# Meng-333/FastDiffSR

Measured on NVIDIA B200. Metric: sr_images_per_s_T20, higher is better.
Workload: dtype fp16

## Files before the change

fastdiffsr_b200/csrc/api.cu:

```cuda
#include <algorithm>
#include <cmath>
#include <cstdarg>
#include <cstdio>
#include <cstdlib>
#include <cstring>
#include <map>
#include <string>
#include <utility>
#include <vector>

#include <cuda_runtime.h>

#include "../../include/fdsr.h"
#include "aux_kernels.cuh"
#include "conv_kernel.cuh"
#include "conv_f32.cuh"
#include "attn_kernel.cuh"
#include "tile_kernels.cuh"

using namespace fdsr;

namespace {

thread_local std::string g_global_error;
// ... 88 lines not shown
  std::string err;
  std::vector<HTensor> tensors;
  std::vector<HConv> convs;
  std::vector<HAttn> attns;
  std::vector<HOp> ops;
  int t_xin = -1, t_last = -1;
  std::map<std::string, std::vector<float>> host_w;
  bool weights_loaded = false;
  DevBuf<uint8_t> d_weights;
  DevBuf<float> d_params;
  DevBuf<float> d_bias;
  int T = 0;
  std::map<std::string, std::vector<double>> tables;
  std::vector<PostCoef> post;
  int B = 0, H = 0, W = 0;
  DevBuf<uint8_t> d_ws;
  size_t ws_bytes = 0;
  size_t stats_off = 0, stats_bytes = 0;
  size_t off_cond = 0, off_x = 0, off_eps = 0, off_sr = 0, off_psum = 0, off_pmax = 0, off_gate = 0,
         off_sp = 0, off_seed = 0;
  std::vector<ConvLayer> h_layers;
  std::vector<F32Layer> f_layers;
  std::vector<F32GnArgs> f_gn;
  std::vector<AttnParams> a_params;
  bool pair = true;
  bool half_tiles = true;
  bool split_n = true;
  bool epi2 = true;
  bool tail_help = true;
  bool resid_mma = true;
  bool up_phases = true;
  bool fused_tail = true;
  bool attn_ref = false;
  DevBuf<float> d_weights32;
  std::vector<size_t> w32_off;
  size_t off_gntab = 0;
  int esize() const { return cfg.dtype == FDSR_DTYPE_FP32 ? 4 : 2; }
  int bands() const { return cfg.out_channel; }
  DevBuf<long long> d_prof;
  bool layers_dirty = true;
  struct BicTab {
    int in, out, ksize;
    DevBuf<int> d_min, d_cnt, d_taps;
  };
  std::vector<BicTab> bic;
  DevBuf<uint8_t> d_bic_tmp;
  DevBuf<unsigned long long> d_metric;
  struct HostSlot {
    uint8_t* h_pin = nullptr;
    size_t h_pin_bytes = 0;
    DevBuf<uint8_t> d_stage;
    size_t in_b = 0, out_b = 0;
    cudaEvent_t computed = nullptr, copied = nullptr;
    bool busy = false;
  };
  static constexpr int kHostSlots = 2;
  HostSlot slot[kHostSlots];
  cudaStream_t copy_stream = nullptr;
  bool use_graph = true;
  DevBuf<PostStep> d_post;
  ConvLayer final_fused{};
  struct GraphEntry {
    int B, H, W;
    bool noise, trace;
    cudaGraphExec_t exec;
    uint64_t used;
// ... 50 lines not shown
}

template <typename... P, typename... A>
int launch(fdsr_ctx* c, void (*kernel)(P...), dim3 grid, dim3 block, size_t smem, cudaStream_t st, A&&... args) {
  kernel<<<grid, block, smem, st>>>(std::forward<A>(args)...);
  return launched(c, cudaSuccess, reinterpret_cast<const void*>(kernel));
}

template <typename T, typename H>
int upload(fdsr_ctx* c, DevBuf<T>& b, const std::vector<H>& host, size_t pad = 0) {
  cudaFree(b.ptr);
  b.ptr = nullptr;
  b.cap = 0;
  CUDA_TRY(c, b.grow(host.size() * sizeof(H) + pad));
  CUDA_TRY(c, cudaMemcpy(b.ptr, host.data(), host.size() * sizeof(H), cudaMemcpyHostToDevice));
  return FDSR_OK;
}

template <typename T>
struct Elem {
  using type = T;
};
template <typename F>
auto with_dtype16(const fdsr_ctx* c, F&& f) {
  return c->cfg.dtype == FDSR_DTYPE_BF16 ? f(Elem<__nv_bfloat16>{}) : f(Elem<__half>{});
}
template <typename F>
auto with_dtype(const fdsr_ctx* c, F&& f) {
  return c->cfg.dtype == FDSR_DTYPE_FP32 ? f(Elem<float>{}) : with_dtype16(c, f);
}

int pad_n(int cout) { return cout <= 16 ? 16 : (cout <= 64 ? 64 : (cout <= 128 ? 128 : 256)); }

constexpr int kOpScheduleFields = 17;

void add_conv(fdsr_ctx* c, const HConv& k) {
  c->convs.push_back(k);
  c->ops.push_back({0, int(c->convs.size()) - 1});
}

int add_tensor(fdsr_ctx* c, const std::string& name, int C, int level, bool stats) {
  HTensor t;
  t.name = name;
  t.C = C;
  t.level = level;
  t.stats = stats;
  c->tensors.push_back(t);
  return int(c->tensors.size()) - 1;
}

std::vector<HTap> taps3x3() {
  std::vector<HTap> v;
  for (int ky = 0; ky < 3; ++ky)
    for (int kx = 0; kx < 3; ++kx) v.push_back({ky, kx, ky * kPatchW + kx});
  return v;
}

int add_res(fdsr_ctx* c, const std::string& name, const std::vector<int>& srcs, int cout, int level,
            const std::string& out_name) {
  const std::string p = "denoise_fn." + name + ".res_block";
  int cin = 0;
  for (int s : srcs) cin += c->tensors[s].C;
  const int th = add_tensor(c, name + ".h", cout, level, true);
  const int to = add_tensor(c, out_name, cout, level, true);
  {
    HConv k;
    k.name = name + ".block1";
// ... 713 lines not shown
        g.C[s2] = t.C;
      }
      if (k.gn_nsrc == 1) {
        g.stats[1] = g.stats[0];
        g.C[1] = 0;
      }
      const HTensor& t0 = c->tensors[k.src[0]];
      g.gn_C = k.gn_C;
      g.groups = c->cfg.norm_groups;
      g.HW = (H >> t0.level) * (W >> t0.level);
      g.sq_scale = stat_sq_scale((long long)g.HW);
      g.eps = 1e-5f;
      g.gamma = c->d_params + k.gamma_off;
      g.beta = c->d_params + k.gamma_off + k.gn_C;
      g.tab = reinterpret_cast<float2*>(c->d_ws + c->off_gntab);
    }
  }
  static_assert(sizeof(F32Layer) <= 4000, "F32Layer must fit the kernel parameter space");
  c->layers_dirty = false;
  return FDSR_OK;
}

int launch_conv_f32(fdsr_ctx* c, int li, int t, cudaStream_t st) {
  const HConv& k = c->convs[li];
  const F32Layer& l = c->f_layers[li];
  if (k.gn_C) {
    const int rc = launch(c, f32_gn_table_kernel, c->B, 256, 0, st, c->f_gn[li]);
    if (rc) return rc;
  }
  const int tiles = c->B * ((l.W + kF32Tile - 1) / kF32Tile) * ((l.H + kF32Tile - 1) / kF32Tile);
  return launch(c, conv_f32_kernel, dim3(tiles, (l.N + kF32NBlk - 1) / kF32NBlk), 256, 0, st, l, t);
}

int upload_layers(fdsr_ctx* c) {
  if (c->cfg.dtype == FDSR_DTYPE_FP32) return upload_layers_f32(c);
  const int B = c->B, H = c->H, W = c->W;
  const bool bf = c->cfg.dtype == FDSR_DTYPE_BF16;
  if (!c->d_prof) {
    CUDA_TRY(c, c->d_prof.grow(size_t(c->num_sms) * kProfRoles * 64));
    CUDA_TRY(c, cudaMemset(c->d_prof, 0, size_t(c->num_sms) * kProfRoles * 64));
  }
  std::vector<ConvLayer> L(c->convs.size());
  for (size_t i = 0; i < c->convs.size(); ++i) {
    const HConv& k = c->convs[i];
    ConvLayer& l = L[i];
    memset(&l, 0, sizeof l);
    const int lvl = k.out >= 0 ? c->tensors[k.out].level : 0;
    l.B = B;
    l.phases = k.phases;
    l.H = (H >> lvl) >> (k.phases == 4 ? 1 : 0);
    l.W = (W >> lvl) >> (k.phases == 4 ? 1 : 0);
    l.tiles_x = (l.W + kTileW - 1) / kTileW;
    const int full_tiles = B * l.tiles_x * ((l.H + kTileH - 1) / kTileH);
    const bool half = c->half_tiles && c->pair && k.mode == kModeNormal && k.ncg == 8 && k.phases == 1 &&
                      k.out_mode == kOutAct && k.N >= 128 && l.tiles_x % 2 == 0 && l.H % 16 == 0 && full_tiles <= c->num_sms;
    l.tile_h = half ? 16 : kTileH;
    l.tiles_y = (l.H + l.tile_h - 1) / l.tile_h;
    l.ntiles = B * k.phases * l.tiles_x * l.tiles_y;
    l.nsplit = (!half && c->split_n && k.out_mode == kOutAct && k.N == 256 && 2 * l.ntiles <= c->num_sms) ? 2 : 1;
    l.n_full = k.N;
    l.N = k.N / l.nsplit;
    l.ncg = k.ncg;
    l.mode = k.mode;
    for (int s = 0; s < k.nsrc; ++s) {
      const HTensor& t = c->tensors[k.src[s]];
      l.src[s].ptr = c->d_ws + t.off;
// ... 53 lines not shown
      bool ok = true;
      if (k.phases == 4)
        for (int ph = 0; ph < 4 && ok; ++ph)
          ok = make_out_map_phase(ph == 0 ? &l.out_map : &l.out_map_ph[ph - 1], l.out, B, l.H, l.W, k.N, ph, bf);
      else if (k.N >= 32)
        ok = make_out_map(&l.out_map, l.out, B, l.H, l.W, k.N, bf);
      if (!ok) return fail(c, FDSR_E_CUDA, "layer %s: tensor maps of the output failed", k.name.c_str());
      l.out_stats = t.stats ? reinterpret_cast<unsigned long long*>(c->d_ws + t.stats_off) : nullptr;
      l.out_sq_scale = float(stat_sq_scale((long long)(H >> t.level) * (W >> t.level)));
      int su = 1;
      while (su < 8 && t.unit % (4 * su) == 0) su *= 2;
      l.out_su = (l.N == 64) ? 1 : su;
    } else {
      l.out = c->d_ws + c->off_eps;
    }
    l.pair = (c->pair && k.pair_ok() && l.a_tma && l.nsplit == 1 && l.tiles_x % 2 == 0) ? 1 : 0;
    l.weights = c->d_weights + (l.pair ? k.w_off2 : k.w_off);
    l.w_half = int32_t(k.w_bytes / 2);
    {
      const int tpi = l.tiles_x * l.tiles_y;
      l.group = (l.N == 64 && tpi % (l.pair ? 4 : 2) == 0) ? 2 : 1;
    }
    {
      bool raw = k.mode == kModeNormal && k.out_mode == kOutAct && l.tile_h == kTileH && l.nsplit == 1 && k.resid < 0;
      for (const HChunk& ch : k.chunks) raw = raw && ch.gn == 0;
      l.epi2 = (c->epi2 && raw) ? 1 : 0;
      if (l.epi2 && l.N <= 128) {
        l.nG = 2;
        l.nR = 0;
        for (int j = 0; j < l.nchunks; ++j) l.chunk[j].ring = 0;
      }
    }
    l.tail2 = (c->tail_help && !l.epi2 && k.out_mode == kOutAct && l.N >= 64) ? 1 : 0;
    l.prof = c->d_prof;
    l.flags = reinterpret_cast<unsigned int*>(c->d_ws + kOffFlags);
  }
  static_assert(sizeof(ConvLayer) <= 4000, "ConvLayer must fit the kernel parameter space");
  c->final_fused = L.back();
  c->final_fused.out_mode = kOutPosterior;
  c->final_fused.post = c->d_post;
  c->final_fused.x_state = reinterpret_cast<float*>(c->d_ws + c->off_x);
  c->final_fused.xin = c->d_ws + c->tensors[c->t_xin].off;
  c->final_fused.args = reinterpret_cast<const SampleArgs*>(c->d_ws + c->off_seed);
  c->h_layers = L;
  const int rc = upload_attn(c);
  if (rc) return rc;
  c->layers_dirty = false;
  return FDSR_OK;
}

int ensure_layers(fdsr_ctx* c) { return c->layers_dirty ? upload_layers(c) : FDSR_OK; }

template <int N, typename T>
cudaError_t set_conv_attr() {
  cudaError_t e = cudaFuncSetAttribute(conv_gemm_kernel<N, T, false>, cudaFuncAttributeMaxDynamicSharedMemorySize,
                                       ConvCfg<N>::kSmemBytes);
  if constexpr (N >= 64) {
    if (e == cudaSuccess)
      e = cudaFuncSetAttribute(conv_gemm_kernel<N, T, true>, cudaFuncAttributeMaxDynamicSharedMemorySize,
                               ConvCfg<N>::kSmemBytes);
  }
  return e;
}
template <typename T>
cudaError_t set_conv_attrs() {
  cudaError_t e = set_conv_attr<16, T>();
// ... 418 lines not shown
  return launch(c, set_args_kernel, 1, 1, 0, st, reinterpret_cast<SampleArgs*>(c->d_tiled.ptr),
                SampleArgs{seed, c->image0, noise, trace});
}
}

extern "C" {

const char* fdsr_global_error(void) { return g_global_error.c_str(); }
const char* fdsr_last_error(const fdsr_ctx* ctx) { return ctx ? ctx->err.c_str() : g_global_error.c_str(); }

int fdsr_create(const fdsr_config* cfg, fdsr_ctx** out) {
  if (!cfg || !out) return fail(nullptr, FDSR_E_INVALID, "null argument");
  int ndev = 0;
  if (cudaGetDeviceCount(&ndev) != cudaSuccess || ndev == 0)
    return fail(nullptr, FDSR_E_CUDA, "no CUDA device: libfdsr has no CPU fallback");
  fdsr_ctx* c = new fdsr_ctx();
  c->cfg = *cfg;
  cudaGetDevice(&c->device);
  cudaDeviceProp prop;
  if (cudaGetDeviceProperties(&prop, c->device) != cudaSuccess || prop.major != 10) {
    delete c;
    return fail(nullptr, FDSR_E_CUDA, "libfdsr needs an sm_100 (B200) device");
  }
  c->num_sms = prop.multiProcessorCount;
  c->pair = env_hook("FDSR_PAIR", c->pair);
  c->half_tiles = env_hook("FDSR_HALF_TILES", c->half_tiles);
  c->split_n = env_hook("FDSR_SPLIT_N", c->split_n);
  c->epi2 = env_hook("FDSR_EPI2", c->epi2);
  c->tail_help = env_hook("FDSR_TAIL_HELP", c->tail_help);
  c->resid_mma = env_hook("FDSR_RESID_MMA", c->resid_mma);
  c->up_phases = env_hook("FDSR_UP_PHASES", c->up_phases);
  c->fused_tail = env_hook("FDSR_FUSED_TAIL", c->fused_tail);
  c->attn_ref = env_hook("FDSR_ATTN_REF", c->attn_ref);
  if (cfg->dtype < FDSR_DTYPE_FP16 || cfg->dtype > FDSR_DTYPE_FP32) {
    delete c;
    return fail(nullptr, FDSR_E_INVALID, "dtype must be FDSR_DTYPE_FP16, FDSR_DTYPE_BF16 or FDSR_DTYPE_FP32");
  }
  const int rc = build_plan(c);
  if (rc) {
    g_global_error = c->err;
    delete c;
    return rc;
  }
  const cudaError_t ae = cfg->dtype == FDSR_DTYPE_FP32 ? cudaSuccess : with_dtype16(c, [&](auto e) {
    using T = typename decltype(e)::type;
    cudaError_t r = set_conv_attrs<T>();
    for (const HAttn& a : c->attns)
      if (r == cudaSuccess && a.kind == 1)
        r = cudaFuncSetAttribute(attn_core<T>(a.C).first, cudaFuncAttributeMaxDynamicSharedMemorySize,
                                 attn_core<T>(a.C).second);
    return r;
  });
  if (ae != cudaSuccess) {
    delete c;
    return fail(nullptr, FDSR_E_CUDA, "cudaFuncSetAttribute(max dynamic smem) failed: %s", cudaGetErrorString(ae));
  }
  *out = c;
  return FDSR_OK;
}

int fdsr_destroy(fdsr_ctx* c) {
  if (!c) return FDSR_OK;
  c->drop_graphs();
  for (auto& sl : c->slot) {
    if (sl.h_pin) cudaFreeHost(sl.h_pin);
    if (sl.computed) cudaEventDestroy(sl.computed);
// ... 499 lines not shown
  return nm.c_str();
}
static double op_flops(const fdsr_ctx* c, int32_t i, bool executed) {
  if (!c || i < 0 || i >= int(c->ops.size()) || c->ops[i].kind != 0) return 0.0;
  const HConv& k = c->convs[c->ops[i].idx];
  const int lvl = k.out >= 0 ? c->tensors[k.out].level : 0;
  return 2.0 * conv_macs(k, executed) * k.cout * double(c->B) * (c->H >> lvl) * (c->W >> lvl);
}
double fdsr_debug_op_flops(const fdsr_ctx* c, int32_t i) { return op_flops(c, i, false); }
double fdsr_debug_op_flops_executed(const fdsr_ctx* c, int32_t i) { return op_flops(c, i, true); }

int fdsr_debug_op_schedule(fdsr_ctx* c, int32_t i, int32_t* out_host, int32_t cap) {
  if (!c || !out_host) return fail(c, FDSR_E_INVALID, "null argument");
  if (i < 0 || i >= int(c->ops.size()) || c->ops[i].kind != 0) return fail(c, FDSR_E_INVALID, "op %d is not a conv", i);
  if (c->cfg.dtype == FDSR_DTYPE_FP32) return fail(c, FDSR_E_INVALID, "the fp32 parity mode has no tile schedule");
  if (c->layers_dirty || c->h_layers.empty()) return fail(c, FDSR_E_STATE, "run fdsr_unet_forward at the shape first");
  if (cap < kOpScheduleFields) return fail(c, FDSR_E_INVALID, "capacity too small (%d needed)", kOpScheduleFields);
  const ConvLayer& l = c->h_layers[c->ops[i].idx];
  const int grid = conv_grid(c, l);
  const int cs = l.pair ? 2 : 1, ngroups = l.ntiles / cs / l.group, nclusters = grid / cs / l.nsplit;
  const int tq = ngroups / nclusters, tr = ngroups - tq * nclusters, tpi = l.tiles_x * l.tiles_y;
  int max_tiles = 0, spans_image = 0, spans_phase = 0;
  for (int cid = 0; cid < nclusters; ++cid) {
    const int units = tq + (cid < tr ? 1 : 0);
    if (units == 0) continue;
    const int tb = (cid * tq + (cid < tr ? cid : tr)) * l.group, te = tb + units * l.group;
    max_tiles = std::max(max_tiles, te - tb);
    const int b0 = tb * cs / tpi, b1 = ((te - 1) * cs + cs - 1) / tpi;
    spans_image |= b0 / l.phases != b1 / l.phases;
    for (int b = b0; b < b1 && l.phases > 1; ++b) spans_phase |= b / l.phases == (b + 1) / l.phases;
  }
  const int32_t v[kOpScheduleFields] = {l.N,     l.pair,  l.tile_h, l.nsplit, l.group,  grid,        l.ntiles,    max_tiles,
                                        l.epi2,  l.tail2, l.nR,     l.nG,     l.phases, l.a_tma,     spans_image, spans_phase,
                                        l.nchunks};
  std::copy(v, v + kOpScheduleFields, out_host);
  return kOpScheduleFields;
}

int fdsr_debug_profile_unet(fdsr_ctx* c, int32_t t, int32_t reps, float* ms_out_host, int32_t cap, void* stream) {
  if (!c || !ms_out_host) return fail(c, FDSR_E_INVALID, "null argument");
  int rc = check_ready(c);
  if (rc) return rc;
  if (!c->d_ws) return fail(c, FDSR_E_STATE, "run fdsr_unet_forward / fdsr_sample once first");
  const int nops = int(c->ops.size());
  if (cap < nops) return fail(c, FDSR_E_INVALID, "capacity too small");
  cudaStream_t st = static_cast<cudaStream_t>(stream);
  rc = ensure_layers(c);
  if (rc) return rc;
  std::vector<cudaEvent_t> ev(size_t(nops) * 2 * reps);
  for (auto& e : ev) CUDA_TRY(c, cudaEventCreate(&e));
  for (int r = 0; r < reps; ++r) {
    CUDA_TRY(c, cudaMemsetAsync(c->d_ws + c->stats_off, 0, c->stats_bytes, st));
    for (int i = 0; i < nops; ++i) {
      const HOp& op = c->ops[i];
      CUDA_TRY(c, cudaEventRecord(ev[(size_t(r) * nops + i) * 2], st));
      rc = with_dtype(c, [&](auto e) {
        using T = typename decltype(e)::type;
        return op.kind == 0 ? launch_conv<T>(c, op.idx, t, st) : launch_attn<T>(c, op.idx, st);
      });
      if (rc) return rc;
      CUDA_TRY(c, cudaEventRecord(ev[(size_t(r) * nops + i) * 2 + 1], st));
    }
  }
  CUDA_TRY(c, cudaStreamSynchronize(st));
  const int r0 = reps >= 4 ? reps / 2 : 0;
  for (int i = 0; i < nops; ++i) {
    double acc = 0.0;
// ... 112 lines not shown
```

fastdiffsr_b200/csrc/conv_desc.h:

```cpp
#pragma once
#include <cstdint>
#include <cuda.h>

namespace fdsr {

constexpr int kMaxChunks = 24;
constexpr int kMaxTaps = 9;
constexpr int kMaxSrc = 3;

constexpr int kTileH = 32;
constexpr int kTileW = 8;
constexpr int kPatchW = kTileW + 2;
constexpr int kPatchH = kTileH + 2;
constexpr int kPatchPos = kPatchW * kPatchH;
constexpr int kPlanePos = 341;
constexpr int kPlaneBytes = kPlanePos * 16;
constexpr int kPlaneBytesTma = 344 * 16;
constexpr int kPatchBytesSw = kPatchPos * 128;
constexpr int kAStageBytes = 8 * kPlaneBytes;
static_assert(kPatchBytesSw <= kAStageBytes && kAStageBytes % 128 == 0, "A stage too small");

enum ConvMode : int32_t {
  kModeNormal = 0,
  kModeUp2x = 1,
// ... 47 lines not shown
  CUtensorMap in_map[kMaxSrc];
  CUtensorMap in_map_c[kMaxSrc];
  CUtensorMap out_map_ph[3];
  ConvSrc src[kMaxSrc];
  ConvChunk chunk[kMaxChunks];
  int32_t nchunks;
  int32_t ncg;
  int32_t mode;
  int32_t nG, nR;
  int32_t a_tma;
  int32_t B, H, W;
  int32_t N;
  int32_t n_full;
  int32_t nsplit;
  int32_t gn_C;
  int32_t gn_nsrc;
  int32_t gn_groups;
  const float* gamma;
  const float* beta;
  float gn_eps;
  const float* bias;
  int32_t bias_tstride;
  const void* resid;
  void* out;
  unsigned long long* out_stats;
  float out_sq_scale;
  double gn_inv_sum, gn_inv_sq;
  int32_t out_su;
  int32_t out_mode;
  int32_t out_c;
  const uint8_t* weights;
  int32_t pair;
  int32_t w_half;
  int32_t phases;
  int32_t epi2;
  int32_t tail2;
  int32_t tile_h;
  int32_t tiles_x, tiles_y, ntiles;
  int32_t group;
  const PostStep* post;
  float* x_state;
  void* xin;
  const SampleArgs* args;
  unsigned int* flags;
  long long* prof;
};

}
```

fastdiffsr_b200/csrc/conv_kernel.cuh:

```cuda
#pragma once
#include "conv_desc.h"
#include "ptx.cuh"
#include "sampler_math.cuh"

namespace fdsr {

constexpr int kConvThreads = 640;
constexpr int kProdWarps = 10;
constexpr int kProdThreads = kProdWarps * 32;
constexpr int kMaxUnits = 9;
constexpr int kEpiWarps = 8;
constexpr int kEpiThreads = kEpiWarps * 32;
constexpr int kMaxGnC = 512;
constexpr double kStatScale = 16777216.0;
__host__ __device__ inline double stat_sq_scale(long long hw) {
  int lg = 0;
  while ((1LL << lg) < hw) ++lg;
  int e = 30 - lg;
  e = e < 4 ? 4 : (e > 24 ? 24 : e);
  return double(1LL << e);
}

template <int N>
struct ConvCfg {
  static constexpr int kAccStride = N < 32 ? 32 : N;
  static constexpr int kAccCols = 2 * kAccStride;
  static constexpr int kNumAcc = (2 * kAccCols <= 512) ? 2 : 1;
  static constexpr int kNumAccMax = 2;
  static constexpr bool kStatsInTmem = (N == 64);
  static constexpr int kStatCol0 = kNumAcc * kAccCols;
  static constexpr int kTmemNeed = kNumAcc * kAccCols + (kStatsInTmem ? 2 * N : 0);
  static constexpr int kTmemCols =
      kTmemNeed <= 32 ? 32 : (kTmemNeed <= 64 ? 64 : (kTmemNeed <= 128 ? 128 : (kTmemNeed <= 256 ? 256 : 512)));
  static constexpr int kBStageBytes = N < 32 ? 9 * N * 128 : (N == 64 ? 24576 : 32768);
  static constexpr int kAStages = N >= 256 ? 2 : 3;
  static constexpr int kBStages = N >= 256 ? 3 : 2;
  static constexpr int kRStageBytes = kTileH * kTileW * 128;
  static constexpr int kASlots = N == 64 ? 4 : kAStages;
  static constexpr int kABytes =
      N == 64 ? (2 * kAStageBytes + 2 * kRStageBytes > 3 * kAStageBytes ? 2 * kAStageBytes + 2 * kRStageBytes
                                                                        : 3 * kAStageBytes)
              : kAStages * kAStageBytes;
  static constexpr int kNcb = N < 32 ? 1 : N / 32;
  static constexpr int kRow = N < 32 ? 32 : N;
  static constexpr int kOffA = 0;
  static constexpr int kOffB = kOffA + kABytes;
  static constexpr int kOffTable = kOffB + kBStages * kBStageBytes;
  static constexpr int kOffBias = kOffTable + kMaxGnC * 8;
  static constexpr int kOffTstat = kOffBias + 256 * 4;
  static constexpr int kOffBar = kOffTstat + kEpiWarps * kRow * 4;
  static constexpr int kNumBar = 3 * kASlots + 2 * kBStages + 2 * kNumAccMax + (kASlots + kBStages + kNumAccMax);
  static constexpr int kOffTmem = kOffBar + kNumBar * 8;
  static constexpr int kOffStage = ((kOffTmem + 16 + 1023) / 1024) * 1024;
  static constexpr int kSmemBytes = kOffStage + (N < 32 ? 0 : kEpiWarps * 2048) + (N >= 256 ? 7 * 2048 : 0);
  static_assert(kSmemBytes <= 232448, "exceeds the 227 KB of dynamic shared memory per CTA");
};

template <typename T>
struct Cvt;
template <>
struct Cvt<__half> {
  static constexpr int kFmt = 0;
  __device__ static __forceinline__ float2 unpack(uint32_t u) {
    return __half22float2(*reinterpret_cast<const __half2*>(&u));
  }
  __device__ static __forceinline__ uint32_t pack(float a, float b) {
    __half2 h = __floats2half2_rn(a, b);
    return *reinterpret_cast<uint32_t*>(&h);
  }
  __device__ static __forceinline__ uint32_t pack_store(float a, float b) {
    uint32_t r;
    asm("cvt.rn.satfinite.f16x2.f32 %0, %1, %2;" : "=r"(r) : "f"(b), "f"(a));
    return r;
  }
};
template <>
struct Cvt<__nv_bfloat16> {
  static constexpr int kFmt = 1;
  __device__ static __forceinline__ float2 unpack(uint32_t u) {
    return __bfloat1622float2(*reinterpret_cast<const __nv_bfloat162*>(&u));
  }
  __device__ static __forceinline__ uint32_t pack(float a, float b) {
    __nv_bfloat162 h = __floats2bfloat162_rn(a, b);
    return *reinterpret_cast<uint32_t*>(&h);
// ... 159 lines not shown
#define PROF_PARAM
#define PROF_ARG
#endif

template <bool kPair>
constexpr int kTileStep = kPair ? 2 : 1;

struct TileWalk {
  int b, ty, tx, step;
  const ConvLayer* L;
  TileWalk() = default;
  __device__ __forceinline__ TileWalk(int t, const ConvLayer& layer, int step_) : step(step_), L(&layer) {
    b = t / (L->tiles_x * L->tiles_y);
    ty = (t - b * L->tiles_x * L->tiles_y) / L->tiles_x;
    tx = t - (b * L->tiles_y + ty) * L->tiles_x;
  }
  __device__ __forceinline__ void advance() {
    if ((tx += step) >= L->tiles_x) {
      tx -= L->tiles_x;
      if (++ty == L->tiles_y) { ty = 0; ++b; }
    }
  }
  __device__ __forceinline__ TileWalk peek_next() const { TileWalk n = *this; n.advance(); return n; }
};

struct StageRing {
  int slot = 0, phase = 0;
  __device__ __forceinline__ void advance(int n) { if (++slot == n) { slot = 0; phase ^= 1; } }
};

template <int N>
struct ConvBars {
  using Cfg = ConvCfg<N>;
  static constexpr int kA = Cfg::kASlots, kB = 2 * kA, kAcc = kB + 2 * Cfg::kBStages, kRaw = kAcc + 2 * Cfg::kNumAccMax,
                       kRelay = kRaw + kA;
  uint32_t bar0;
  __device__ __forceinline__ uint32_t a_full(int s) const { return bar0 + 8u * s; }
  __device__ __forceinline__ uint32_t a_empty(int s) const { return bar0 + 8u * (kA + s); }
  __device__ __forceinline__ uint32_t b_full(int s) const { return bar0 + 8u * (kB + s); }
  __device__ __forceinline__ uint32_t b_empty(int s) const { return bar0 + 8u * (kB + Cfg::kBStages + s); }
  __device__ __forceinline__ uint32_t acc_full(int s) const { return bar0 + 8u * (kAcc + s); }
  __device__ __forceinline__ uint32_t acc_empty(int s) const { return bar0 + 8u * (kAcc + Cfg::kNumAccMax + s); }
  __device__ __forceinline__ uint32_t raw_full(int s) const { return bar0 + 8u * (kRaw + s); }
  __device__ __forceinline__ uint32_t pa_full(int s) const { return bar0 + 8u * (kRelay + s); }
  __device__ __forceinline__ uint32_t pb_full(int s) const { return bar0 + 8u * (kRelay + kA + s); }
  __device__ __forceinline__ uint32_t pacc_empty(int s) const { return bar0 + 8u * (kRelay + kA + Cfg::kBStages + s); }
};

template <int N>
struct ConvSched {
  int tile_begin, tile_end;
  int tile_first;
  TileWalk first;
  uint32_t crank;
  int TH, nacc, taps_per_stage, n_off, nG, nR;
  bool two_mt;
  uint32_t acc_cols, blob, gblob;
  __device__ __forceinline__ uint32_t slot_off(int slot) const {
    return uint32_t(slot < nG ? slot * kAStageBytes : nG * kAStageBytes + (slot - nG) * ConvCfg<N>::kRStageBytes);
  }
};

template <int N, typename T, bool kPair>
__device__ __forceinline__ void mma_role(const ConvLayer& L, const ConvSched<N>& S, const ConvBars<N>& bars,
                                         uint32_t tmem, uint8_t* smem PROF_PARAM) {
  using Cfg = ConvCfg<N>;
  constexpr int NB = kPair ? N / 2 : N;
  const int lane = threadIdx.x & 31;
  const uint32_t sA = smem_u32(smem + Cfg::kOffA), sB = smem_u32(smem + Cfg::kOffB);
  const uint32_t idesc_raw = make_idesc_f16(kPair ? 256 : 128, N, Cvt<T>::kFmt);
  const uint32_t idesc_gn = make_idesc_f16(kPair ? 256 : 128, N, Cvt<GnOperand<T>>::kFmt);
  const bool leader = S.crank == 0;
  const bool sw = L.a_tma == 1;
  const uint32_t a_hi_full = sw ? (((kPatchW * 128) >> 4) | (1u << 14) | (2u << 29)) : (((kPatchW * 16) >> 4) | (1u << 14));
  const uint32_t a_hi_cen = ((kTileW * 128) >> 4) | (1u << 14) | (2u << 29);
  const uint32_t b_hi = (128u >> 4) | (1u << 14);
  const uint32_t plane16 = L.a_tma == 2 ? uint32_t(kPlaneBytesTma >> 4) : uint32_t(kPlaneBytes >> 4);
  const uint32_t a_lo0 = ((sw ? 1u : plane16) << 16) + ((sA & 0x3FFFFu) >> 4);
  const uint32_t kstep = sw ? 2u : 2u * plane16;
  const int pos_sh = sw ? 3 : 0;
  const uint32_t mt1_full = uint32_t(16 * kPatchW) << pos_sh;
  const uint32_t b_lo0 = (uint32_t((NB * 16) >> 4) << 16) + ((sB & 0x3FFFFu) >> 4);
  const int ksteps = L.ncg >> 1;
  StageRing ga, ra, bst, acc;
  int bq = 0;
  TileWalk walk = S.first;
  auto pair_sync = [&](uint32_t relay_bar, uint32_t use_parity) {
    if constexpr (kPair) {
      if (leader) mbar_wait(relay_bar, use_parity);
      else if (lane == 0) mbar_arrive_remote(relay_bar, 0);
      __syncwarp();
    }
  };
  PROF_DECL;
  for (int tile = S.tile_begin; tile < S.tile_end; ++tile) {
    mbar_wait(bars.acc_empty(acc.slot), acc.phase ^ 1);
    pair_sync(bars.pacc_empty(acc.slot), acc.phase);
    PROF_MARK(0);
    tc_fence_after();
    const uint32_t d0 = tmem + acc.slot * S.acc_cols;
    const uint32_t phoff = L.phases > 1 ? uint32_t(((walk.b >> 1) & 1) * kPatchW + (walk.b & 1)) << pos_sh : 0u;
    walk.advance();
    for (int c = 0; c < L.nchunks; ++c) {
      const ConvChunk& ck = L.chunk[c];
      const int ntaps = ck.ntaps;
      const bool r1 = ck.ring != 0;
      const int as = r1 ? S.nG + ra.slot : ga.slot, aph = r1 ? ra.phase : ga.phase;
      const uint32_t idesc = ck.gn != 0 ? idesc_gn : idesc_raw;
      mbar_wait(bars.a_full(as), aph);
      pair_sync(bars.pa_full(as), aph);
      PROF_MARK(1);
      const uint32_t a_stage = a_lo0 + (S.slot_off(as) >> 4);
      const bool cen = ck.center != 0;
      const uint32_t a_hi = cen ? a_hi_cen : a_hi_full;
      const uint32_t mt1 = cen ? uint32_t(16 * kTileW) << 3 : mt1_full;
      for (int tp0 = 0; tp0 < ntaps;) {
        const int g = ntaps - tp0 < S.taps_per_stage - bq ? ntaps - tp0 : S.taps_per_stage - bq;
        if (bq == 0) {
          mbar_wait(bars.b_full(bst.slot), bst.phase);
          pair_sync(bars.pb_full(bst.slot), bst.phase);
        }
        PROF_MARK(2);
        tc_fence_after();
        const bool stage_done = bq + g == S.taps_per_stage;
        if (leader && elect_one()) {
          if (tile == S.tile_begin && c == 0 && tp0 == 0) PROF_TS(4);
          uint32_t b_lo = b_lo0 + bst.slot * (Cfg::kBStageBytes >> 4) + bq * (S.blob >> 4);
          for (int tg = 0; tg < g; ++tg, b_lo += S.blob >> 4) {
            const uint32_t a_lo = a_stage + (cen ? 0u : (uint32_t(ck.tap_pos[tp0 + tg]) << pos_sh) + phoff);
            const uint32_t accum0 = (c | tp0 | tg) == 0 ? 0u : 1u;
            auto issue = [&](int ks) {
              const uint64_t bd = (uint64_t(b_hi) << 32) | (b_lo + ks * 2 * NB);
              const uint64_t ad0 = (uint64_t(a_hi) << 32) | (a_lo + ks * kstep);
              const uint64_t ad1 = (uint64_t(a_hi) << 32) | (a_lo + ks * kstep + mt1);
              if constexpr (kPair) {
                umma_f16_pair(d0, ad0, bd, idesc, ks ? 1u : accum0);
                if (S.two_mt) umma_f16_pair(d0 + Cfg::kAccStride, ad1, bd, idesc, ks ? 1u : accum0);
              } else {
                umma_f16(d0, ad0, bd, idesc, ks ? 1u : accum0);
                if (S.two_mt) umma_f16(d0 + Cfg::kAccStride, ad1, bd, idesc, ks ? 1u : accum0);
              }
            };
            if (ksteps == 4) {
#pragma unroll
              for (int ks = 0; ks < 4; ++ks) issue(ks);
            } else {
              for (int ks = 0; ks < ksteps; ++ks) issue(ks);
            }
          }
          auto commit = [&](uint32_t bar) {
            if constexpr (kPair) umma_commit_pair(bar);
            else umma_commit(bar);
          };
          if (stage_done) commit(bars.b_empty(bst.slot));
          if (tp0 + g >= ntaps) commit(bars.a_empty(as));
          if (tp0 + g >= ntaps && c == L.nchunks - 1) {
            commit(bars.acc_full(acc.slot));
            if (tile + 1 == S.tile_end) PROF_TS(5);
          }
        }
        __syncwarp();
        PROF_MARK(3);
        tp0 += g;
        bq += g;
        if (stage_done) {
          bq = 0;
          bst.advance(Cfg::kBStages);
        }
      }
      if (r1) ra.advance(S.nR);
      else ga.advance(S.nG);
    }
    acc.advance(S.nacc);
  }
  if (lane == 0) PROF_FLUSH(0);
}

template <int N, typename T, bool kPair>
__device__ __forceinline__ void loader_role(const ConvLayer& L, const ConvSched<N>& S, const ConvBars<N>& bars,
                                            uint8_t* smem) {
  using Cfg = ConvCfg<N>;
  const uint32_t sA = smem_u32(smem + Cfg::kOffA), sB = smem_u32(smem + Cfg::kOffB);
  const uint32_t patch_bytes = uint32_t((S.TH + 2) * kPatchW) * 128u, cen_bytes = uint32_t(S.TH) * kTileW * 128u;
  const bool tma_in = L.a_tma != 0;
  const int ncg = L.ncg, n_full = L.n_full;
  if (tma_in) asm volatile("griddepcontrol.wait;" ::: "memory");
  const int total = (S.tile_end - S.tile_begin) * L.nchunks;
  int a_next = tma_in ? 0 : total, a_c = 0;
  StageRing a_ga, a_ra;
  TileWalk a_walk = S.first;
  int taps_tile = 0;
  for (int c = 0; c < L.nchunks; ++c) taps_tile += L.chunk[c].ntaps;
  const int total_taps = (S.tile_end - S.tile_begin) * taps_tile;
  int b_q = 0, b_qq = 0;
  StageRing bst;
  const uint8_t* const w0 = L.weights + (kPair ? size_t(S.crank) * size_t(L.w_half) : size_t(S.n_off) * 16);
  const int phsh = L.phases > 1 ? 2 : 0;
  const size_t ph_stride = L.phases > 1 ? size_t(taps_tile) * (kPair ? S.blob : S.gblob) : 0;
  TileWalk w_walk = S.first;
  while (a_next < total || b_q < total_taps) {
    bool progress = false;
    if (a_next < total) {
      const bool a_r1 = L.chunk[a_c].ring != 0;
      const int a_as = a_r1 ? S.nG + a_ra.slot : a_ga.slot;
      const uint32_t ok = mbar_test(bars.a_empty(a_as), (a_r1 ? a_ra.phase : a_ga.phase) ^ 1) ? 1u : 0u;
      if (__shfl_sync(0xffffffffu, ok, 0)) {
        if (elect_one()) {
          const ConvChunk& ak = L.chunk[a_c];
          const uint32_t dst = sA + S.slot_off(a_as);
          const int a_b = a_walk.b, a_ty = a_walk.ty, a_tx = a_walk.tx;
          if (L.a_tma == 2) {
            const uint32_t bar = bars.a_full(a_as);
            mbar_arrive_cnt(bar, kProdWarps - 1);
            mbar_arrive_expect_tx(bar, 2 * kPatchPos * 16);
            tma_load_4d(&L.in_map[ak.src], dst, bar, ak.c0, a_tx * kTileW - 1, a_ty * kTileH - 1, a_b);
            tma_load_4d(&L.in_map[ak.src], dst + kPlaneBytesTma, bar, ak.c0 + 8, a_tx * kTileW - 1, a_ty * kTileH - 1, a_b);
          } else if (ak.gn != 0) {
            mbar_arrive_expect_tx(bars.raw_full(a_as), patch_bytes);
            tma_load_4d(&L.in_map[ak.src], dst, bars.raw_full(a_as), ak.c0, a_tx * kTileW - 1, a_ty * S.TH - 1, a_b >> phsh);
          } else {
            const uint32_t bar = bars.a_full(a_as);
            mbar_arrive_cnt(bar, kProdWarps - 1);
            if (L.mode == kModeS2D) {
              mbar_arrive_expect_tx(bar, patch_bytes);
              tma_load_4d(&L.in_map_c[ak.src], dst, bar, ak.c0, 2 * (a_tx * kTileW - 1) + (ak.parity & 1),
                          2 * (a_ty * S.TH - 1) + (ak.parity >> 1), a_b);
            } else if (ak.center != 0) {
              mbar_arrive_expect_tx(bar, cen_bytes);
              tma_load_4d(&L.in_map_c[ak.src], dst, bar, ak.c0, a_tx * kTileW, a_ty * S.TH, a_b >> phsh);
            } else {
              mbar_arrive_expect_tx(bar, patch_bytes);
              tma_load_4d(&L.in_map[ak.src], dst, bar, ak.c0, a_tx * kTileW - 1, a_ty * S.TH - 1, a_b >> phsh);
            }
          }
        }
        __syncwarp();
        ++a_next;
        if (a_r1) a_ra.advance(S.nR);
        else a_ga.advance(S.nG);
        if (++a_c == L.nchunks) {
          a_c = 0;
          a_walk.advance();
        }
        progress = true;
      }
    }
    if (b_q < total_taps) {
      const uint32_t ok = mbar_test(bars.b_empty(bst.slot), bst.phase ^ 1) ? 1u : 0u;
      if (__shfl_sync(0xffffffffu, ok, 0)) {
        const int g = total_taps - b_q < S.taps_per_stage ? total_taps - b_q : S.taps_per_stage;
        if (elect_one()) {
          mbar_arrive_expect_tx(bars.b_full(bst.slot), uint32_t(g) * S.blob);
          const uint32_t dst0 = sB + bst.slot * Cfg::kBStageBytes;
          if (L.nsplit == 1) {
            int rem = g, qq = b_qq;
            TileWalk t = w_walk;
            uint32_t dst = dst0;
            while (rem > 0) {
              const int n = rem < taps_tile - qq ? rem : taps_tile - qq;
              bulk_g2s(dst, w0 + size_t(t.b & 3) * ph_stride + size_t(qq) * S.blob, uint32_t(n) * S.blob, bars.b_full(bst.slot));
              dst += uint32_t(n) * S.blob;
              rem -= n;
              qq += n;
              if (qq == taps_tile) {
                qq = 0;
                t.advance();
              }
            }
          } else {
            int qq = b_qq;
            TileWalk t = w_walk;
            for (int tg = 0; tg < g; ++tg) {
              const uint8_t* wt = w0 + size_t(t.b & 3) * ph_stride + size_t(qq) * S.gblob;
              const uint32_t dst = dst0 + uint32_t(tg) * S.blob;
              for (int cgi = 0; cgi < ncg; ++cgi)
                bulk_g2s(dst + uint32_t(cgi) * N * 16, wt + size_t(cgi) * n_full * 16, N * 16, bars.b_full(bst.slot));
              if (++qq == taps_tile) {
                qq = 0;
                t.advance();
              }
            }
          }
        }
        __syncwarp();
        bst.advance(Cfg::kBStages);
        b_q += g;
        for (b_qq += g; b_qq >= taps_tile; b_qq -= taps_tile) w_walk.advance();
        progress = true;
      }
    }
    if (!progress) __nanosleep(32);
  }
}

template <int N, typename T, bool kPair>
__device__ __forceinline__ void producer_role(const ConvLayer& L, const ConvSched<N>& S, const ConvBars<N>& bars,
                                              uint8_t* smem PROF_PARAM) {
  using Cfg = ConvCfg<N>;
  constexpr int kAStages = Cfg::kAStages;
  const int warp = threadIdx.x >> 5, lane = threadIdx.x & 31;
  const int pw = warp < 4 ? warp - 2 : warp - 10;
  const int pidx = pw * 32 + lane;
  __builtin_assume(pidx >= 0 && pidx < kProdThreads);
  const int H = L.H, W = L.W, TH = S.TH;
  const int npos = (TH + 2) * kPatchW;
  const uint32_t sA = smem_u32(smem + Cfg::kOffA);
  float2* table = reinterpret_cast<float2*>(smem + Cfg::kOffTable);
  __half* table_h = reinterpret_cast<__half*>(table);
  int cur_b = -1;
  TileWalk walk = S.first;
  PROF_DECL;

  const int cpg = L.gn_C > 0 ? L.gn_C / L.gn_groups : 2, ppg = cpg >> 1, p0 = L.src[0].C >> 1;
  float ga[2] = {0.f, 0.f}, be[2] = {0.f, 0.f};
#pragma unroll
  for (int j = 0; j < 2; ++j) {
    const int c = pidx + j * kProdThreads;
    if (c < L.gn_C) {
// ... 521 lines not shown
  if (et == 0) PROF_TS(6);
  if (et == 0) PROF_FLUSH(1);
  (void)et;
}

template <int N, typename T, bool kPair>
__global__ void __launch_bounds__(kConvThreads, 1)
conv_gemm_kernel(const __grid_constant__ ConvLayer L, int t_step) {
  using Cfg = ConvCfg<N>;
  PROF_T0;
  constexpr int kASlots = Cfg::kASlots;
  constexpr int kTStep = kTileStep<kPair>;
  extern __shared__ __align__(1024) uint8_t smem[];
  const int tid = threadIdx.x, warp = tid >> 5, lane = tid & 31;
  const ConvBars<N> bars{smem_u32(smem + Cfg::kOffBar)};
  uint32_t* tmem_slot = reinterpret_cast<uint32_t*>(smem + Cfg::kOffTmem);
  const uint32_t crank = kPair ? cluster_ctarank() : 0u;

  if (warp == 1) {
    if (lane < kMaxSrc && L.src[lane].ptr != nullptr && L.a_tma != 0) {
      prefetch_tensormap(&L.in_map[lane]);
      if (L.a_tma == 1) prefetch_tensormap(&L.in_map_c[lane]);
    }
    if (lane == 8 && N >= 32 && L.out_mode == kOutAct) prefetch_tensormap(&L.out_map);
    if (lane >= 9 && lane < 12 && L.phases > 1) prefetch_tensormap(&L.out_map_ph[lane - 9]);
  }
  if (tid == 0) {
    for (int s = 0; s < kASlots; ++s) {
      mbar_init(bars.a_full(s), kProdWarps);
      mbar_init(bars.a_empty(s), 1);
      mbar_init(bars.raw_full(s), 1);
      mbar_init(bars.pa_full(s), 1);
    }
    for (int s = 0; s < Cfg::kBStages; ++s) {
      mbar_init(bars.b_full(s), 1);
      mbar_init(bars.b_empty(s), 1);
      mbar_init(bars.pb_full(s), 1);
    }
    for (int s = 0; s < Cfg::kNumAccMax; ++s) {
      mbar_init(bars.acc_full(s), 1);
      mbar_init(bars.acc_empty(s), L.epi2 ? 2 * kEpiWarps : kEpiWarps);
      mbar_init(bars.pacc_empty(s), 1);
    }
    mbar_init_fence();
  }
  if (warp == 0) tmem_alloc<Cfg::kTmemCols, kPair>(smem_u32(tmem_slot));
  tc_fence_before();
  __syncthreads();
  if (kPair) cluster_arrive();
  tc_fence_after();
  const uint32_t tmem = *tmem_slot;
  if (kPair && warp == 0) cluster_wait();
  if (kPair && tid == 0) {
    uint32_t ra, other;
    asm volatile("mapa.shared::cluster.u32 %0, %1, %2;" : "=r"(ra) : "r"(smem_u32(tmem_slot)), "r"(crank ^ 1u));
    asm volatile("ld.shared::cluster.u32 %0, [%1];" : "=r"(other) : "r"(ra) : "memory");
    if (other != tmem) asm volatile("trap;");
  }
  if (tid == 0) PROF_TS(0);
  asm volatile("griddepcontrol.launch_dependents;");
  const bool epi_team2 = L.epi2 != 0 && warp >= 4 + kEpiWarps;
  const bool is_producer = (warp == 2 || warp == 3 || warp >= 4 + kEpiWarps) && !epi_team2;
  bool epi_role = (warp >= 4 && warp < 4 + kEpiWarps) || epi_team2;
  bool tail_helper = false;
  if (warp != 1 && !is_producer) asm volatile("griddepcontrol.wait;" ::: "memory");
  if (tid == 0) PROF_TS(1);

  const int tgroup = L.group;
  const int ngroups = (L.ntiles / kTStep) / tgroup;
  const int nsplit = L.nsplit;
  const int part = int(blockIdx.x) % nsplit;
  const int nclusters = int(gridDim.x / kTStep) / nsplit, cid = int(blockIdx.x / kTStep) / nsplit;
  const int tq = ngroups / nclusters, tr = ngroups - tq * nclusters;
  const int unit_begin = cid * tq + (cid < tr ? cid : tr);
  const int my_units = tq + (cid < tr ? 1 : 0);
  ConvSched<N> S;
  S.tile_begin = unit_begin * tgroup;
  S.tile_end = S.tile_begin + my_units * tgroup;
  S.tile_first = S.tile_begin * kTStep + int(crank);
  S.first = TileWalk(S.tile_first, L, kTStep);
  S.crank = crank;
  S.TH = L.tile_h;
  S.two_mt = S.TH == kTileH;
  S.nacc = S.two_mt ? Cfg::kNumAcc : Cfg::kNumAccMax;
  S.acc_cols = S.two_mt ? Cfg::kAccCols : Cfg::kAccStride;
  S.blob = uint32_t(L.ncg) * (kPair ? N / 2 : N) * 16;
  S.gblob = uint32_t(L.ncg) * uint32_t(L.n_full) * 16;
  S.taps_per_stage = int(Cfg::kBStageBytes / S.blob) < kMaxTaps ? int(Cfg::kBStageBytes / S.blob) : kMaxTaps;
  S.n_off = part * N;
  S.nG = L.nG;
  S.nR = L.nR;

  if (warp == 0) {
    mma_role<N, T, kPair>(L, S, bars, tmem, smem PROF_ARG);
  } else if (warp == 1) {
    loader_role<N, T, kPair>(L, S, bars, smem);
  } else if (!epi_role) {
    producer_role<N, T, kPair>(L, S, bars, smem PROF_ARG);
    if (L.tail2 != 0 && warp >= 4 + kEpiWarps && S.tile_end > S.tile_begin) {
      tail_helper = true;
      epi_role = true;
    }
  }
  if (epi_role) epilogue_role<N, T, kPair>(L, S, bars, tmem, smem, t_step, epi_team2, tail_helper PROF_ARG);

  tc_fence_before();
  if (kPair && warp != 0) cluster_wait();
  __syncthreads();
  if (kPair) cluster_sync_all();
  if (tid == 0) PROF_TS(7);
  if (warp == 0) tmem_dealloc<Cfg::kTmemCols, kPair>(tmem);
}

}
```

fastdiffsr_b200/engine.py:

```python
from __future__ import annotations

import ctypes as C

import numpy as np
import torch

from . import _lib
from ._lib import FdsrConfig, FdsrError, FdsrOverflowError

_DTYPES = {"auto": _lib.DTYPE_FP16, "fp16": _lib.DTYPE_FP16, "float16": _lib.DTYPE_FP16, "bf16": _lib.DTYPE_BF16, "bfloat16": _lib.DTYPE_BF16,
           "fp32": _lib.DTYPE_FP32, "float32": _lib.DTYPE_FP32}


def _ptr(t):
    return C.c_void_p(t.data_ptr()) if t is not None else C.c_void_p(0)


class Engine:
    def __init__(self, unet_cfg: dict, device, dtype: str = "fp16"):
        self.lib = _lib.load()
        self.device = torch.device(device)
        if self.device.type != "cuda":
            raise FdsrError("fastdiffsr_b200 runs on CUDA (sm_100a) devices only; there is no CPU fallback")
        mults = list(unet_cfg["channel_multiplier"])
# ... 220 lines not shown
        return out

    def sse_u8(self, a, b):
        a, b = self._img(a, "a"), self._img(b, "b")
        B, _, H, W = a.shape
        out = torch.empty(B, dtype=torch.float64, device=self.device)
        self._call("fdsr_sse_u8", _ptr(a), _ptr(b), B, H, W, _ptr(out), self._stream())
        return out

    def metrics_u8(self, a, b, scale: float = 4.0):
        a, b = self._img(a, "a"), self._img(b, "b")
        B, _, H, W = a.shape
        out = torch.empty((B, 4), dtype=torch.float64, device=self.device)
        self._call("fdsr_metrics_u8", _ptr(a), _ptr(b), B, H, W, float(scale), _ptr(out), self._stream())
        return out

    def tensor_names(self):
        n = self.lib.fdsr_debug_num_tensors(self._h)
        return [self.lib.fdsr_debug_tensor_name(self._h, i).decode() for i in range(n)]

    def read_tensor(self, name: str, B: int, max_elems: int):
        buf = torch.empty(max_elems, dtype=torch.float32, device=self.device)
        c, h, w = C.c_int32(), C.c_int32(), C.c_int32()
        self._call("fdsr_debug_read_tensor", name.encode(), _ptr(buf), max_elems, C.byref(c), C.byref(h), C.byref(w),
                   self._stream())
        n = B * c.value * h.value * w.value
        return buf[:n].view(B, c.value, h.value, w.value)

    def op_flops_executed(self):
        n = self.lib.fdsr_debug_num_ops(self._h)
        return [float(self.lib.fdsr_debug_op_flops_executed(self._h, i)) for i in range(n)]

    OP_SCHEDULE_FIELDS = ("N", "pair", "tile_h", "nsplit", "group", "grid", "ntiles", "max_tiles", "epi2", "tail2", "nR",
                          "nG", "phases", "a_tma", "spans_image", "spans_phase", "nchunks")

    def op_names(self):
        return [self.lib.fdsr_debug_op_name(self._h, i).decode() for i in range(self.lib.fdsr_debug_num_ops(self._h))]

    def op_schedule(self, op: int):
        buf = (C.c_int32 * len(self.OP_SCHEDULE_FIELDS))()
        n = self._call("fdsr_debug_op_schedule", op, buf, len(buf))
        return dict(zip(self.OP_SCHEDULE_FIELDS, buf[:n]))

    def profile_unet(self, t: int, reps: int = 3):
        n = self.lib.fdsr_debug_num_ops(self._h)
        ms = (C.c_float * n)()
        self._call("fdsr_debug_profile_unet", t, reps, ms, n, self._stream())
        return [(self.lib.fdsr_debug_op_name(self._h, i).decode(), float(ms[i]),
                 float(self.lib.fdsr_debug_op_flops(self._h, i))) for i in range(n)]

    def role_cycles(self, op: int, t: int = 0):
        n = 148 * 40 * 2
        buf = (C.c_int64 * n)()
        m = self._call("fdsr_debug_role_cycles", op, t, buf, n, self._stream())
        return np.array(buf[:m], dtype=np.int64).reshape(-1, 5, 8)

    def timeline(self, t: int = 0, reps: int = 3):
        nops = int(self.lib.fdsr_debug_num_ops(self._h))
        nsm = torch.cuda.get_device_properties(self.device).multi_processor_count
        out = np.zeros((nops, nsm, 5, 8), dtype=np.int64)
        self._call("fdsr_debug_timeline", t, reps, out.ctypes.data_as(C.POINTER(C.c_int64)), out.size, self._stream())
        return out

    def launch_count(self):
        return int(self.lib.fdsr_launch_count(self._h))

    def unet_flops(self):
# ... 11 lines not shown
```

Baseline: 168.2.

## Keep N=64 pair-conv weights resident in shared memory or use three weight stages

Adds a per-layer shared-memory plan for paired N=64 convolutions. If all of a layer's weight taps fit in the weight stage buffers, they are loaded once per persistent CTA and kept resident, which drops the per-tile weight reloads and the empty/full barrier handshakes. Otherwise, when there is no residual ring and three accumulator-group slots, weights get three stages placed in unused patch memory to deepen the weight pipeline. This adds runtime stage parameters, an extra barrier slot, and the risk of aliasing the patch buffers.

```diff
diff --git a/fastdiffsr_b200/csrc/api.cu b/fastdiffsr_b200/csrc/api.cu
--- a/fastdiffsr_b200/csrc/api.cu
+++ b/fastdiffsr_b200/csrc/api.cu
@@ -144,6 +144,7 @@
   bool up_phases = true;
   bool fused_tail = true;
   bool attn_ref = false;
+  bool smem_plan = true;
   DevBuf<float> d_weights32;
   std::vector<size_t> w32_off;
   size_t off_gntab = 0;
@@ -260,7 +261,7 @@
 
 int pad_n(int cout) { return cout <= 16 ? 16 : (cout <= 64 ? 64 : (cout <= 128 ? 128 : 256)); }
 
-constexpr int kOpScheduleFields = 17;
+constexpr int kOpScheduleFields = 19;
 
 void add_conv(fdsr_ctx* c, const HConv& k) {
   c->convs.push_back(k);
@@ -1040,6 +1041,35 @@
   return launch(c, conv_f32_kernel, dim3(tiles, (l.N + kF32NBlk - 1) / kF32NBlk), 256, 0, st, l, t);
 }
 
+template <int N>
+void default_weight_stages(ConvLayer& l) {
+  l.nB = ConvCfg<N>::kBStages;
+  l.b_off = ConvCfg<N>::kOffB;
+  l.b_stage = ConvCfg<N>::kBStageBytes;
+}
+
+void plan_weights(ConvLayer& l, bool plan) {
+  switch (l.N) {
+    case 16: default_weight_stages<16>(l); break;
+    case 64: default_weight_stages<64>(l); break;
+    case 128: default_weight_stages<128>(l); break;
+    default: default_weight_stages<256>(l); break;
+  }
+  using Cfg = ConvCfg<64>;
+  if (!plan || !l.pair || l.N != 64 || l.phases != 1 || l.mode != kModeNormal) return;
+  int taps = 0;
+  for (int j = 0; j < l.nchunks; ++j) taps += l.chunk[j].ntaps;
+  const int blob = l.ncg * (l.N / 2) * 16;
+  if (taps * blob <= Cfg::kBStages * Cfg::kBStageBytes) {
+    l.w_res = 1;
+  } else if (l.nR == 0 && l.nG == 3) {
+    l.nB = 3;
+    l.b_off = 3 * kAStageBytes;
+    l.b_stage = (Cfg::kOffTable - l.b_off) / 3 / blob * blob;
+    static_assert(3 <= Cfg::kBSlots && (3 * kAStageBytes) % 16 == 0, "weight stages in the patch memory");
+  }
+}
+
 int upload_layers(fdsr_ctx* c) {
   if (c->cfg.dtype == FDSR_DTYPE_FP32) return upload_layers_f32(c);
   const int B = c->B, H = c->H, W = c->W;
@@ -1159,6 +1189,7 @@
       }
     }
     l.tail2 = (c->tail_help && !l.epi2 && k.out_mode == kOutAct && l.N >= 64) ? 1 : 0;
+    plan_weights(l, c->smem_plan);
     l.prof = c->d_prof;
     l.flags = reinterpret_cast<unsigned int*>(c->d_ws + kOffFlags);
   }
@@ -1643,6 +1674,7 @@
   c->up_phases = env_hook("FDSR_UP_PHASES", c->up_phases);
   c->fused_tail = env_hook("FDSR_FUSED_TAIL", c->fused_tail);
   c->attn_ref = env_hook("FDSR_ATTN_REF", c->attn_ref);
+  c->smem_plan = env_hook("FDSR_SMEM_PLAN", c->smem_plan);
   if (cfg->dtype < FDSR_DTYPE_FP16 || cfg->dtype > FDSR_DTYPE_FP32) {
     delete c;
     return fail(nullptr, FDSR_E_INVALID, "dtype must be FDSR_DTYPE_FP16, FDSR_DTYPE_BF16 or FDSR_DTYPE_FP32");
@@ -2208,7 +2240,7 @@
   }
   const int32_t v[kOpScheduleFields] = {l.N,     l.pair,  l.tile_h, l.nsplit, l.group,  grid,        l.ntiles,    max_tiles,
                                         l.epi2,  l.tail2, l.nR,     l.nG,     l.phases, l.a_tma,     spans_image, spans_phase,
-                                        l.nchunks};
+                                        l.nchunks, l.w_res, l.nB};
   std::copy(v, v + kOpScheduleFields, out_host);
   return kOpScheduleFields;
 }
diff --git a/fastdiffsr_b200/csrc/conv_desc.h b/fastdiffsr_b200/csrc/conv_desc.h
--- a/fastdiffsr_b200/csrc/conv_desc.h
+++ b/fastdiffsr_b200/csrc/conv_desc.h
@@ -103,6 +103,8 @@
   const uint8_t* weights;
   int32_t pair;
   int32_t w_half;
+  int32_t nB, b_off, b_stage;
+  int32_t w_res;
   int32_t phases;
   int32_t epi2;
   int32_t tail2;
diff --git a/fastdiffsr_b200/csrc/conv_kernel.cuh b/fastdiffsr_b200/csrc/conv_kernel.cuh
--- a/fastdiffsr_b200/csrc/conv_kernel.cuh
+++ b/fastdiffsr_b200/csrc/conv_kernel.cuh
@@ -35,6 +35,7 @@
   static constexpr int kBStageBytes = N < 32 ? 9 * N * 128 : (N == 64 ? 24576 : 32768);
   static constexpr int kAStages = N >= 256 ? 2 : 3;
   static constexpr int kBStages = N >= 256 ? 3 : 2;
+  static constexpr int kBSlots = N == 64 ? 3 : kBStages;
   static constexpr int kRStageBytes = kTileH * kTileW * 128;
   static constexpr int kASlots = N == 64 ? 4 : kAStages;
   static constexpr int kABytes =
@@ -49,7 +50,7 @@
   static constexpr int kOffBias = kOffTable + kMaxGnC * 8;
   static constexpr int kOffTstat = kOffBias + 256 * 4;
   static constexpr int kOffBar = kOffTstat + kEpiWarps * kRow * 4;
-  static constexpr int kNumBar = 3 * kASlots + 2 * kBStages + 2 * kNumAccMax + (kASlots + kBStages + kNumAccMax);
+  static constexpr int kNumBar = 3 * kASlots + 2 * kBSlots + 2 * kNumAccMax + (kASlots + kBSlots + kNumAccMax);
   static constexpr int kOffTmem = kOffBar + kNumBar * 8;
   static constexpr int kOffStage = ((kOffTmem + 16 + 1023) / 1024) * 1024;
   static constexpr int kSmemBytes = kOffStage + (N < 32 ? 0 : kEpiWarps * 2048) + (N >= 256 ? 7 * 2048 : 0);
@@ -275,19 +276,19 @@
 template <int N>
 struct ConvBars {
   using Cfg = ConvCfg<N>;
-  static constexpr int kA = Cfg::kASlots, kB = 2 * kA, kAcc = kB + 2 * Cfg::kBStages, kRaw = kAcc + 2 * Cfg::kNumAccMax,
+  static constexpr int kA = Cfg::kASlots, kB = 2 * kA, kAcc = kB + 2 * Cfg::kBSlots, kRaw = kAcc + 2 * Cfg::kNumAccMax,
                        kRelay = kRaw + kA;
   uint32_t bar0;
   __device__ __forceinline__ uint32_t a_full(int s) const { return bar0 + 8u * s; }
   __device__ __forceinline__ uint32_t a_empty(int s) const { return bar0 + 8u * (kA + s); }
   __device__ __forceinline__ uint32_t b_full(int s) const { return bar0 + 8u * (kB + s); }
-  __device__ __forceinline__ uint32_t b_empty(int s) const { return bar0 + 8u * (kB + Cfg::kBStages + s); }
+  __device__ __forceinline__ uint32_t b_empty(int s) const { return bar0 + 8u * (kB + Cfg::kBSlots + s); }
   __device__ __forceinline__ uint32_t acc_full(int s) const { return bar0 + 8u * (kAcc + s); }
   __device__ __forceinline__ uint32_t acc_empty(int s) const { return bar0 + 8u * (kAcc + Cfg::kNumAccMax + s); }
   __device__ __forceinline__ uint32_t raw_full(int s) const { return bar0 + 8u * (kRaw + s); }
   __device__ __forceinline__ uint32_t pa_full(int s) const { return bar0 + 8u * (kRelay + s); }
   __device__ __forceinline__ uint32_t pb_full(int s) const { return bar0 + 8u * (kRelay + kA + s); }
-  __device__ __forceinline__ uint32_t pacc_empty(int s) const { return bar0 + 8u * (kRelay + kA + Cfg::kBStages + s); }
+  __device__ __forceinline__ uint32_t pacc_empty(int s) const { return bar0 + 8u * (kRelay + kA + Cfg::kBSlots + s); }
 };
 
 template <int N>
@@ -310,7 +311,8 @@
   using Cfg = ConvCfg<N>;
   constexpr int NB = kPair ? N / 2 : N;
   const int lane = threadIdx.x & 31;
-  const uint32_t sA = smem_u32(smem + Cfg::kOffA), sB = smem_u32(smem + Cfg::kOffB);
+  const bool wres = L.w_res != 0;
+  const uint32_t sA = smem_u32(smem + Cfg::kOffA), sB = smem_u32(smem + L.b_off);
   const uint32_t idesc_raw = make_idesc_f16(kPair ? 256 : 128, N, Cvt<T>::kFmt);
   const uint32_t idesc_gn = make_idesc_f16(kPair ? 256 : 128, N, Cvt<GnOperand<T>>::kFmt);
   const bool leader = S.crank == 0;
@@ -359,7 +361,7 @@
       const uint32_t mt1 = cen ? uint32_t(16 * kTileW) << 3 : mt1_full;
       for (int tp0 = 0; tp0 < ntaps;) {
         const int g = ntaps - tp0 < S.taps_per_stage - bq ? ntaps - tp0 : S.taps_per_stage - bq;
-        if (bq == 0) {
+        if (bq == 0 && (!wres || tile == S.tile_begin)) {
           mbar_wait(bars.b_full(bst.slot), bst.phase);
           pair_sync(bars.pb_full(bst.slot), bst.phase);
         }
@@ -368,7 +370,7 @@
         const bool stage_done = bq + g == S.taps_per_stage;
         if (leader && elect_one()) {
           if (tile == S.tile_begin && c == 0 && tp0 == 0) PROF_TS(4);
-          uint32_t b_lo = b_lo0 + bst.slot * (Cfg::kBStageBytes >> 4) + bq * (S.blob >> 4);
+          uint32_t b_lo = b_lo0 + bst.slot * (uint32_t(L.b_stage) >> 4) + bq * (S.blob >> 4);
           for (int tg = 0; tg < g; ++tg, b_lo += S.blob >> 4) {
             const uint32_t a_lo = a_stage + (cen ? 0u : (uint32_t(ck.tap_pos[tp0 + tg]) << pos_sh) + phoff);
             const uint32_t accum0 = (c | tp0 | tg) == 0 ? 0u : 1u;
@@ -395,7 +397,7 @@
             if constexpr (kPair) umma_commit_pair(bar);
             else umma_commit(bar);
           };
-          if (stage_done) commit(bars.b_empty(bst.slot));
+          if (stage_done && !wres) commit(bars.b_empty(bst.slot));
           if (tp0 + g >= ntaps) commit(bars.a_empty(as));
           if (tp0 + g >= ntaps && c == L.nchunks - 1) {
             commit(bars.acc_full(acc.slot));
@@ -408,7 +410,7 @@
         bq += g;
         if (stage_done) {
           bq = 0;
-          bst.advance(Cfg::kBStages);
+          if (!wres) bst.advance(L.nB);
         }
       }
       if (r1) ra.advance(S.nR);
@@ -423,7 +425,8 @@
 __device__ __forceinline__ void loader_role(const ConvLayer& L, const ConvSched<N>& S, const ConvBars<N>& bars,
                                             uint8_t* smem) {
   using Cfg = ConvCfg<N>;
-  const uint32_t sA = smem_u32(smem + Cfg::kOffA), sB = smem_u32(smem + Cfg::kOffB);
+  const bool wres = L.w_res != 0;
+  const uint32_t sA = smem_u32(smem + Cfg::kOffA), sB = smem_u32(smem + L.b_off);
   const uint32_t patch_bytes = uint32_t((S.TH + 2) * kPatchW) * 128u, cen_bytes = uint32_t(S.TH) * kTileW * 128u;
   const bool tma_in = L.a_tma != 0;
   const int ncg = L.ncg, n_full = L.n_full;
@@ -434,7 +437,7 @@
   TileWalk a_walk = S.first;
   int taps_tile = 0;
   for (int c = 0; c < L.nchunks; ++c) taps_tile += L.chunk[c].ntaps;
-  const int total_taps = (S.tile_end - S.tile_begin) * taps_tile;
+  const int total_taps = (wres ? (S.tile_end > S.tile_begin ? 1 : 0) : S.tile_end - S.tile_begin) * taps_tile;
   int b_q = 0, b_qq = 0;
   StageRing bst;
   const uint8_t* const w0 = L.weights + (kPair ? size_t(S.crank) * size_t(L.w_half) : size_t(S.n_off) * 16);
@@ -494,7 +497,7 @@
         const int g = total_taps - b_q < S.taps_per_stage ? total_taps - b_q : S.taps_per_stage;
         if (elect_one()) {
           mbar_arrive_expect_tx(bars.b_full(bst.slot), uint32_t(g) * S.blob);
-          const uint32_t dst0 = sB + bst.slot * Cfg::kBStageBytes;
+          const uint32_t dst0 = sB + bst.slot * uint32_t(L.b_stage);
           if (L.nsplit == 1) {
             int rem = g, qq = b_qq;
             TileWalk t = w_walk;
@@ -526,7 +529,7 @@
           }
         }
         __syncwarp();
-        bst.advance(Cfg::kBStages);
+        bst.advance(L.nB);
         b_q += g;
         for (b_qq += g; b_qq >= taps_tile; b_qq -= taps_tile) w_walk.advance();
         progress = true;
@@ -1114,7 +1117,7 @@
       mbar_init(bars.raw_full(s), 1);
       mbar_init(bars.pa_full(s), 1);
     }
-    for (int s = 0; s < Cfg::kBStages; ++s) {
+    for (int s = 0; s < Cfg::kBSlots; ++s) {
       mbar_init(bars.b_full(s), 1);
       mbar_init(bars.b_empty(s), 1);
       mbar_init(bars.pb_full(s), 1);
@@ -1168,7 +1171,11 @@
   S.acc_cols = S.two_mt ? Cfg::kAccCols : Cfg::kAccStride;
   S.blob = uint32_t(L.ncg) * (kPair ? N / 2 : N) * 16;
   S.gblob = uint32_t(L.ncg) * uint32_t(L.n_full) * 16;
-  S.taps_per_stage = int(Cfg::kBStageBytes / S.blob) < kMaxTaps ? int(Cfg::kBStageBytes / S.blob) : kMaxTaps;
+  S.taps_per_stage = int(L.b_stage / S.blob) < kMaxTaps ? int(L.b_stage / S.blob) : kMaxTaps;
+  if (L.w_res != 0) {
+    S.taps_per_stage = 0;
+    for (int c = 0; c < L.nchunks; ++c) S.taps_per_stage += L.chunk[c].ntaps;
+  }
   S.n_off = part * N;
   S.nG = L.nG;
   S.nR = L.nR;
diff --git a/fastdiffsr_b200/engine.py b/fastdiffsr_b200/engine.py
--- a/fastdiffsr_b200/engine.py
+++ b/fastdiffsr_b200/engine.py
@@ -276,7 +276,8 @@
         return [float(self.lib.fdsr_debug_op_flops_executed(self._h, i)) for i in range(n)]
 
     OP_SCHEDULE_FIELDS = ("N", "pair", "tile_h", "nsplit", "group", "grid", "ntiles", "max_tiles", "epi2", "tail2", "nR",
-                          "nG", "phases", "a_tma", "spans_image", "spans_phase", "nchunks")
+                          "nG", "phases", "a_tma", "spans_image", "spans_phase", "nchunks",
+                          "w_res", "nB")
 
     def op_names(self):
         return [self.lib.fdsr_debug_op_name(self._h, i).decode() for i in range(self.lib.fdsr_debug_num_ops(self._h))]
```

New measurement: 168.0, median of 6. Within noise of the previous version (-0.1%).
